# IsseiMori/lajolla_public

Hardware: AMD Instinct MI355X
Metric: Msamples/sec (whole node), cbox 256spp (higher is better)
Workload: dtype f32; 1 GPU; cbox.xml 512x512 @ 256 spp, path integrator (Lambertian + area light, max_depth -1, rr_depth 5); rng=pcg32, one stream per (pixel, sample), seed 0x853c49e6748fea9b, parallelism=1 GPU, collective=none

## Files before the change

### __graft_entry__.py

```python
import os
import sys

ROOT = os.path.dirname(os.path.abspath(__file__))
if ROOT not in sys.path:
    sys.path.insert(0, ROOT)


def build():
    from lajolla_public_amd import build as b
    lib = b.build_product()
    b.build_oracle()
    b.build_twin()
    b.build_twin_tile()
    b.build_reference_subset()
    import lajolla_public_amd as lj
    lj.load_library()
    assert os.path.exists(lib)


def smoke():
    import numpy as np
    sys.path.insert(0, os.path.join(ROOT, "tests"))
    import lajolla_public_amd as lj
    from helpers import Oracle, random_rays, scene_path
    hs = lj.parse_scene(scene_path("cbox"))
    ctx = lj.Context(0)
    sc = lj.Scene(ctx, hs)
    o = Oracle(hs)
    rays = random_rays(hs, 20000, 3, o)
    hg, ho = lj.intersect(sc, rays["org"], rays["dir"], 0.0, np.inf), o.intersect(rays)
    for f in ("t", "u", "v", "shape_id", "prim_id"):
        assert np.array_equal(hg[f].view(np.uint32), ho[f].view(np.uint32)), f"traversal mismatch in {f}"
    crop, spp = (224, 232, 288, 280), 8
    rc, _, ps, _ = o.render(spp=spp, rng_mode=0, crop=crop, per_sample=True)
    pg = lj.render_samples(sc, crop, spp=spp)
    rel = np.abs(pg - ps).max(axis=-1) / np.maximum(np.abs(ps).max(axis=-1), 1e-3)
    assert rc == 0 and np.median(rel) < 2e-6 and (rel > 1e-3).mean() < 0.02, (np.median(rel), (rel > 1e-3).mean())
    assert abs(pg.mean() / ps.mean() - 1) < 5e-4
    st = sc.stats()
    print(f"smoke ok: {st.samples} samples, K={st.bounce_iterations / st.samples:.3f}, median rel diff {np.median(rel):.2e}, "
          f"diverged {100 * (rel > 1e-3).mean():.2f} %")


if __name__ == "__main__":
    build()
    if len(sys.argv) > 1 and sys.argv[1] == "smoke":
# ... 2 lines not shown
```

### lajolla_public_amd/build.py

```python
import os
import subprocess
import sys
from concurrent.futures import ThreadPoolExecutor

ROOT = os.path.dirname(os.path.dirname(os.path.abspath(__file__)))
CSRC = os.path.join(ROOT, "lajolla_public_amd", "csrc")
_VARIANT = os.environ.get("LJ_VARIANT", "")
BUILD = os.path.join(ROOT, "build" + ("_" + _VARIANT if _VARIANT else ""))
LIB = os.path.join(ROOT, "lajolla_public_amd", "liblajolla_hip" + ("_" + _VARIANT if _VARIANT else "") + ".so")
_SAN = bool(os.environ.get("LJ_SANITIZE"))
_SAN_FLAGS = ["-fsanitize=address,undefined", "-fno-omit-frame-pointer", "-g"] if _SAN else []
ORACLE_LIB = os.path.join(ROOT, "oracle", "_build", "liblj_oracle_asan.so" if _SAN else "liblj_oracle.so")
TWIN_LIB = os.path.join(ROOT, "tests", "twin", "_build", "libljtwin_asan.so" if _SAN else "libljtwin.so")

HOST_SOURCES = ["host/api_host.cpp", "host/scene_xml.cpp", "host/mesh_io.cpp", "host/image_io.cpp", "host/jpeg_decode.cpp", "host/exr_decode.cpp", "host/png_decode.cpp", "host/tga_bmp_decode.cpp", "host/flatten.cpp", "host/bvh.cpp"]
HIP_SOURCES = ["device/kernels.hip", "device/extend8.hip", "device/volpath.hip", "device/api_device.hip", "device/queries.hip", "device/mega.hip", "device/group.hip", "device/tile.hip"]
ARCH = "gfx950"


def _hipcc():
    for c in (os.environ.get("HIPCC"), "/opt/rocm/bin/hipcc", "hipcc"):
        if c and (os.path.isabs(c) and os.path.exists(c) or not os.path.isabs(c)):
            return c
    raise RuntimeError("hipcc not found")
# ... 85 lines not shown


def build_twin(verbose=True):
    src = os.path.join(ROOT, "tests", "twin", "twin.cpp")
    if not os.path.exists(src):
        return None
    os.makedirs(os.path.dirname(TWIN_LIB), exist_ok=True)
    deps = [src] + _headers() + [os.path.join(CSRC, s) for s in ("host/flatten.cpp", "host/bvh.cpp")]
    if _stale(TWIN_LIB, deps):
        if verbose:
            print("[build] compiling the host twin of the device headers (CPU-side tests only)", file=sys.stderr)
        _run(["g++", "-std=c++17", "-O1" if _SAN else "-O2", "-ffp-contract=off"] + _SAN_FLAGS + _host_fma_flag() + ["-fPIC", "-shared", "-Wall", "-Wno-unused-function",
              "-o", TWIN_LIB, src, os.path.join(CSRC, "host/flatten.cpp"), os.path.join(CSRC, "host/bvh.cpp"), "-lpthread"])
    return TWIN_LIB


TWIN_TILE_LIB = os.path.join(ROOT, "tests", "twin_tile", "_build", "libljtwintile_asan.so" if _SAN else "libljtwintile.so")


def build_twin_tile(verbose=True):
    src = os.path.join(ROOT, "tests", "twin_tile", "twin_tile.cpp")
    if not os.path.exists(src):
        return None
    os.makedirs(os.path.dirname(TWIN_TILE_LIB), exist_ok=True)
    deps = [src] + _headers() + [os.path.join(CSRC, s) for s in ("host/flatten.cpp", "host/bvh.cpp")]
    if _stale(TWIN_TILE_LIB, deps):
        if verbose:
            print("[build] compiling the host twin of the per-tile schedule (CPU-side tests only)", file=sys.stderr)
        _run(["g++", "-std=c++17", "-O1" if _SAN else "-O2", "-ffp-contract=off"] + _SAN_FLAGS + _host_fma_flag() + ["-fPIC", "-shared", "-Wall", "-Wno-unused-function",
              "-o", TWIN_TILE_LIB, src, os.path.join(CSRC, "host/flatten.cpp"), os.path.join(CSRC, "host/bvh.cpp"), "-lpthread"])
    return TWIN_TILE_LIB


def build_reference_subset():
    script = os.path.join(ROOT, "oracle", "ref_build.sh")
    if os.path.isdir(os.environ.get("LJ_REFERENCE_ROOT", "/root/reference")):
        _run(["bash", script])


if __name__ == "__main__":
    build_product()
    if "--oracle" in sys.argv or "--all" in sys.argv:
        build_oracle()
    if "--twin" in sys.argv or "--all" in sys.argv:
        build_twin()
        build_twin_tile()
    print(LIB)
```

### lajolla_public_amd/csrc/device/api_device.hip

```cpp
#include "api_internal.h"

namespace {

void set_device(lj_context *ctx) { HIP_CHECK(hipSetDevice(ctx->device)); }

ljd::DQueue carve_queue(void *base, uint32_t cap) {
    ljd::DQueue q{};
    ljd::Rec4 *p = (ljd::Rec4 *)base;
    auto take = [&]() { ljd::Rec4 *r = p; p += cap; return r; };
    q.ro = take(); q.rd = take(); q.rs = take(); q.rh = take(); q.rw = take(); q.rl = take(); q.rn = take(); q.rg = take();
    return q;
}
size_t queue_bytes(uint32_t cap) { return (size_t)cap * kQueueSlotBytes; }

void ensure_queues(lj_context *ctx, uint32_t cap) {
    if (ctx->queue_capacity >= cap) return;
    cap = (cap + 63u) & ~63u;
    ctx->queue_mem.alloc(queue_bytes(cap));
    ctx->queue_capacity = cap;
}

int *ensure_spill(lj_context *ctx, int levels, uint32_t grid) {
    if (levels <= 0) return nullptr;
    const size_t need = (size_t)levels * grid * 256 * sizeof(int);
// ... 162 lines not shown
            ljd::launch_volpath(ds, pass, (uint32_t)total, (uint32_t *)ctx->chunk_counter.p, sc->ecfg, sc->scfg.variant,
                                 (sc->feat_kinds & ~7u) == 0u && !sc->feat_textured && !sc->feat_envmap && !sc->feat_sphere_lights,
                                ensure_spill(ctx, sc->ecfg.spill_levels, (uint32_t)grid), grid, stream);
            HIP_CHECK(hipGetLastError());
            st.samples += total; st.wavefront_steps++;
            if (rgb_dev) ljd::launch_resolve(pass, (uint32_t)np, rgb_dev, stream);
            if (samples_host) {
                HIP_CHECK(hipMemcpyAsync(samples_host + p0 * (uint64_t)plan.spp * 3, ctx->sample_rgb.p, total * 12, hipMemcpyDeviceToHost, stream));
                HIP_CHECK(hipStreamSynchronize(stream));
            }
        }
        HIP_CHECK(hipEventRecord(ctx->ev_end, stream));
        HIP_CHECK(hipEventSynchronize(ctx->ev_end));
        float ms = 0; HIP_CHECK(hipEventElapsedTime(&ms, ctx->ev_begin, ctx->ev_end));
        unsigned long long nb = 0;
        HIP_CHECK(hipMemcpy(&nb, ctx->chunk_counter.p, 8, hipMemcpyDeviceToHost));
        st.render_ms = ms; st.bounce_iterations = nb;
        if (getenv("LJ_VOLPATH_STATS")) {
            unsigned long long h[32];
            HIP_CHECK(hipMemcpy(h, ctx->chunk_counter.p, sizeof(h), hipMemcpyDeviceToHost));
            const char *names[8] = {"node iterations", "leaf steps", "closest calls", "tracking (bounce ray)", "tracking (shadow segment)", "shadow segments", "path steps", "-"};
            for (int k = 0; k < 7; k++) fprintf(stderr, "[volpath stats] %-26s wave events %12llu  lanes active %5.1f %%  per sample %.2f\n", names[k], h[2 + 2 * k], h[2 + 2 * k] ? 100.0 * h[3 + 2 * k] / (64.0 * h[2 + 2 * k]) : 0.0, (double)h[3 + 2 * k] / (double)st.samples);
        }
        return;
    }
    const size_t mega_lds = ljd::mega_smem(sc->dscene, sc->scfg);
    const bool mega_off = getenv("LJ_TUNE_MEGA") && atoi(getenv("LJ_TUNE_MEGA")) == 0;
    if (mega_lds > 0 && !mega_off) {
        const uint64_t pass_samples_max = pix_per_pass * (uint64_t)plan.spp;
        if (ctx->sample_rgb.bytes < pass_samples_max * 12) ctx->sample_rgb.alloc(pass_samples_max * 12);
        if (!ctx->mega_state.p) ctx->mega_state.alloc(64);
        upload_pixel_list(ctx, plan, stream);
        HIP_CHECK(hipEventRecord(ctx->ev_begin, stream));
        int per_cu = ljd::mega_blocks_per_cu(sc->scfg);
        if (const char *e = getenv("LJ_TUNE_MEGA_BLOCKS_PER_CU")) per_cu = std::max(1, atoi(e));
        uint32_t grab_max = 768, grab_min = 192;
        bool grab_fixed = false;
        if (const char *e = getenv("LJ_TUNE_MEGA_GRAB")) { grab_max = (uint32_t)std::max(64, atoi(e)) & ~63u; grab_fixed = true; }
        double mega_ms = 0;
        unsigned long long hstats[5] = {};
        for (uint64_t p0 = 0; p0 < n_pix; p0 += pix_per_pass) {
            const uint64_t np = std::min<uint64_t>(pix_per_pass, n_pix - p0);
            const uint64_t total = np * (uint64_t)plan.spp;
            ljd::DPass pass{};
            pass.pixel_list = (const uint32_t *)ctx->pixel_list.p + p0; pass.n_pixels = (uint32_t)np; ljd::set_pass_divisors(pass, (uint32_t)plan.spp, (uint32_t)sc->flat.cam.width);
            pass.seed = plan.seed; pass.sample_rgb = (float *)ctx->sample_rgb.p;
            HIP_CHECK(hipMemsetAsync(ctx->mega_state.p, 0, 64, stream));
            uint32_t grab = grab_max;
            if (!grab_fixed) {
                uint64_t draws = 16;
                if (const char *e = getenv("LJ_TUNE_MEGA_DRAWS")) draws = (uint64_t)std::max(1, atoi(e));
                const uint64_t waves = (uint64_t)ctx->n_cus * per_cu * 4, per_draw = total / (waves * draws);
                grab = (uint32_t)std::min<uint64_t>(grab_max, std::max<uint64_t>(grab_min, per_draw & ~(uint64_t)63));
            }
            const uint64_t pieces = (total + grab - 1) / grab;
            const int grid = (int)std::max<uint64_t>(1, std::min<uint64_t>((uint64_t)ctx->n_cus * per_cu, (pieces + 3) / 4));
            if (timing) HIP_CHECK(hipEventRecord(ctx->ev_k0, stream));
            ljd::launch_mega(ds, pass, sc->scfg, sc->flat.n_spheres > 0, (uint32_t)total, grab, (uint32_t *)ctx->mega_state.p,
                             (unsigned long long *)((char *)ctx->mega_state.p + 8), grid, stream);
            HIP_CHECK(hipGetLastError());
            if (timing) {
                HIP_CHECK(hipEventRecord(ctx->ev_k1, stream)); HIP_CHECK(hipEventSynchronize(ctx->ev_k1));
                float a = 0; HIP_CHECK(hipEventElapsedTime(&a, ctx->ev_k0, ctx->ev_k1)); mega_ms += a;
            }
            st.mega_launches++; st.wavefront_steps++;
            if (rgb_dev) ljd::launch_resolve(pass, (uint32_t)np, rgb_dev, stream);
            unsigned long long *h = ctx->stats_host;
// ... 394 lines not shown
```

### lajolla_public_amd/csrc/device/api_internal.h

```cpp
#pragma once
#include <hip/hip_runtime.h>
#include "../host/api_common.h"
#include "../host/flatten.h"
#include "dtypes.h"
#include "dconfig.h"
#include <algorithm>
#include <cstdlib>
#include <cstring>
#include <memory>
#include <string>
#include <vector>

namespace ljd {
ShadeConfig shade_config(size_t n_prims, size_t n_materials, size_t n_lights, size_t n_light_tris, size_t n_light_tri_cdf, size_t n_images3, size_t n_images1, size_t n_env_marg);
int shade_variant(uint32_t kinds, bool textured, bool envmap, bool sphere_lights);
ExtendConfig extend_config(int n_nodes, int n_prims, int bvh_depth, int n_spheres, int n_nodes8, int bvh8_depth, bool open_scene);
int max_stack_depth();
void launch_extend(const DScene &sc, const DQueue &q, const DBlockState *blocks, uint32_t grid, uint32_t seg, uint32_t *work, const uint32_t *chunk_list, uint32_t parity, const ExtendConfig &cfg, int *spill, unsigned long long *stats, hipStream_t s);
bool shade_sorts_segments(const ShadeConfig &cfg);
void launch_shade(const DScene &sc, const DPass &pass, const DQueue &q, const DQueue &qo, uint32_t *sort_perm, uint8_t *sort_keys, DBlockState *blocks, uint32_t n_blocks, uint32_t seg, const ShadeConfig &cfg, uint32_t *work, uint32_t *chunk_list, uint32_t parity, uint32_t extend_waves, hipStream_t s);
void launch_resolve(const DPass &pass, uint32_t n_pixels, float *rgb, hipStream_t s);
size_t tail_smem(const ExtendConfig &ecfg, const ShadeConfig &scfg);
void launch_tail(const DScene &sc, const DPass &pass, const DQueue &q, DBlockState *blocks, uint32_t n_blocks, uint32_t seg, const ExtendConfig &ecfg, const ShadeConfig &scfg, int *spill, hipStream_t s);
void launch_aux(const DScene &sc, const uint32_t *pixel_list, uint32_t n_pixels, int integrator, float *rgb, const ExtendConfig &cfg, int *spill, int grid, hipStream_t s);
void launch_volpath(const DScene &sc, const DPass &pass, uint32_t n_samples, uint32_t *counters, const ExtendConfig &cfg, int shade_variant, bool plain, int *spill, int grid, hipStream_t s);
int volpath_blocks_per_cu(const DScene &sc);
void launch_trace_rays(const DScene &sc, const void *rays, long long n, void *hits, unsigned char *occ, const ExtendConfig &cfg, int *spill, int grid, hipStream_t s);
size_t mega_smem(const DScene &sc, const ShadeConfig &scfg);
int mega_blocks_per_cu(const ShadeConfig &scfg);
void launch_mega(const DScene &sc, const DPass &pass, const ShadeConfig &scfg, bool spheres, uint32_t n_samples, uint32_t grab, uint32_t *sample_counter, unsigned long long *stats, int grid, hipStream_t s);
void launch_trace_rays_scan(const DScene &sc, const void *rays, long long n, void *hits, unsigned char *occ, int grid, hipStream_t s);
size_t tile_cursor_bytes(bool vol);
void launch_tile_init(bool vol, void *cursors, const uint32_t *tiles, uint32_t n_tiles, uint64_t seed, hipStream_t s);
int tile_grid(uint32_t n_tiles, uint32_t lanes);
void launch_tile(bool vol, const DScene &sc, const DTileJob &job, void *cursors, uint32_t lanes, uint32_t budget, uint32_t *alive, const ExtendConfig &cfg, int *spill, hipStream_t s);
void tile_cursor_stats(bool vol, const void *cursors_host, uint32_t n, unsigned long long out[5]);
}

using lj::LjError;

#define HIP_CHECK(expr) do { hipError_t _e = (expr); if (_e != hipSuccess) \
    throw LjError(LJ_ERR_DEVICE, std::string(#expr) + " failed: " + hipGetErrorString(_e)); } while (0)

struct DevBuf {
    void *p = nullptr; size_t bytes = 0;
    void alloc(size_t n) { release(); if (n) { HIP_CHECK(hipMalloc(&p, n)); bytes = n; } }
    void release() { if (p) { (void)hipFree(p); p = nullptr; bytes = 0; } }
    ~DevBuf() { release(); }
    DevBuf() = default; DevBuf(const DevBuf &) = delete; DevBuf &operator=(const DevBuf &) = delete;
};

template <typename T> inline void upload(DevBuf &b, const std::vector<T> &v, hipStream_t s) {
    b.alloc(((std::max<size_t>(v.size(), 1) * sizeof(T)) + 31) & ~(size_t)15);
    if (!v.empty()) HIP_CHECK(hipMemcpyAsync(b.p, v.data(), v.size() * sizeof(T), hipMemcpyHostToDevice, s));
}

static constexpr size_t kQueueSlotBytes = 128;
static constexpr uint32_t kMaxBlocks = 8192;

static constexpr uint32_t kMaxLanes = 8;
struct lj_context {
    int device = 0;
// ... 33 lines not shown
```

### lajolla_public_amd/csrc/device/dshade.h

```cpp
#pragma once
#include "dmath.h"
#include "dconfig.h"

namespace ljd {

template <uint32_t KINDS, bool TEXTURED, bool ENVMAP, bool SPHERE_LIGHTS>
struct ShadeFeat {
    static constexpr uint32_t kinds = KINDS;
    static constexpr bool textured = TEXTURED, envmap = ENVMAP, sphere_lights = SPHERE_LIGHTS;
    static constexpr bool kind(int k) { return ((KINDS >> k) & 1u) != 0u; }
};
using FeatAll = ShadeFeat<0x1ffu, true, true, true>;
using FeatLambert = ShadeFeat<0x001u, false, false, false>;
using FeatPlastic = ShadeFeat<0x003u, false, false, true>;
using FeatLambertTex = ShadeFeat<0x001u, true, false, true>;
using FeatClassic = ShadeFeat<0x007u, true, true, true>;
using FeatDisney = ShadeFeat<0x101u, true, true, false>;
template <class Fn> inline void with_shade_variant(int v, Fn &&fn) {
    switch (v) {
        case 0: fn(FeatLambert{}); break;
        case 1: fn(FeatPlastic{}); break;
        case 2: fn(FeatLambertTex{}); break;
        case 3: fn(FeatClassic{}); break;
        case 4: fn(FeatDisney{}); break;
// ... 710 lines not shown
    }
    if (Ft::kind(1) && m.kind == 1) {
        f3 Ks = tex3<Ft>(sc, m, 1, vx), Kd = tex3<Ft>(sc, m, 0, vx);
        float lS = luminance(Ks), lR = luminance(Kd);
        if (lS + lR <= 0.0f) return s;
        float spec_prob = lS / (lS + lR);
        if (rw < spec_prob) {
            float roughness = clampf(tex1<Ft>(sc, m, 2, vx), 0.01f, 1.0f);
            f3 hm = to_world(frame, sample_visible_normals(to_local(frame, dir_in), roughness * roughness, r0, r1));
            s.dir_out = normalize(-dir_in + hm * (2.0f * dot(dir_in, hm)));
            s.roughness = roughness;
        } else s.dir_out = to_world(frame, sample_cos_hemisphere(r0, r1));
        s.valid = true;
        return s;
    }
    return s;
}

LJ_HD bool material_supported(int kind) { return kind >= 0 && kind <= 8; }

struct PathState {
    f3 org, dir;
    float ht, hu, hv; int32_t hcode;
    f3 sdir; float stfar;
    f3 W; float rr, p2;
    f3 rad, nee;
    uint32_t sample; uint64_t rng;
    float eta_scale, spread;
    uint32_t flags;
};

struct ShadeCounters { uint32_t bounces, closest, shadow, done; };

LJ_HD void generate_path(const DScene &sc, const DPass &pass, uint32_t sample_id, PathState &ps) {
    const uint32_t p = fast_div(sample_id, pass.by_spp), s = sample_id - p * pass.spp;
    const uint32_t pixel = pass.pixel_list[p];
    const int y = (int)fast_div(pixel, pass.by_width), x = (int)(pixel - (uint32_t)y * (uint32_t)sc.cam.width);
    const uint64_t stream = (uint64_t)pixel * pass.spp + s;
    const uint64_t inc = pcg32_inc(stream);
    uint64_t st = pcg32_init(stream, pass.seed);
    const float jy = pcg32_real(st, inc);
    const float jx = pcg32_real(st, inc);
    ps.org = ld3(sc.cam.org);
    ps.dir = camera_primary_dir(sc.cam, x, y, jx, jy);
    ps.sdir = mk3(0, 0, 0); ps.stfar = 0.0f;
    ps.W = mk3(1, 1, 1); ps.rr = 1.0f; ps.p2 = -1.0f;
    ps.rad = mk3(0, 0, 0); ps.nee = mk3(0, 0, 0);
    ps.sample = sample_id; ps.rng = st;
    ps.eta_scale = 1.0f; ps.spread = sc.init_spread;
    ps.flags = 2u;
}

template <class Ft, bool DEFER_RR>
LJ_HD bool shade_path_body(const DScene &sc, uint64_t inc, PathState &ps, ShadeCounters &cnt) {
    if (ps.hcode & HIT_VIS_BIT) ps.rad = ps.rad + ps.nee;
    const bool primary = ps.p2 < 0.0f;
    if (ps.flags & PF_NO_EXT) return false;
    const int gprim = (ps.hcode & 0x3fffffff) - 1;
    const uint32_t nv_prev = ps.flags & 0xffffu;
    if (gprim < 0) {
        if (Ft::envmap && sc.envmap_light_id >= 0) {
            const DLight &E = sc.lights[sc.envmap_light_id];
            f3 L = light_emission<Ft>(sc, E, -ps.dir, mk3(0, 0, 0));
            if (primary) ps.rad = ps.rad + L;
            else {
                float p1 = E.pmf * pdf_point_on_light<Ft>(sc, E, mk3(0, 0, 0), -ps.dir, ps.org);
                float p2 = ps.p2;
                float w2 = (p2 * p2) / (p1 * p1 + p2 * p2);
                ps.rad = ps.rad + ps.W * L * w2;
            }
        }
        return false;
    }
    DVertex vx = build_vertex(sc, ps.org, ps.dir, ps.ht, ps.hu, ps.hv, gprim, primary ? ps.spread : 0.0f);
    if (vx.light_id >= 0) {
        const DLight &EL = sc.lights[vx.light_id];
        f3 L = light_emission<Ft>(sc, EL, -ps.dir, vx.gn);
        if (primary) ps.rad = ps.rad + L;
        else {
            f3 dv = vx.position - ps.org;
            float G = fabsf(dot(ps.dir, vx.gn)) / dot(dv, dv);
            float p2 = ps.p2 * G;
            float p1 = EL.pmf * pdf_point_on_light<Ft>(sc, EL, vx.position, vx.gn, ps.org);
// ... 80 lines not shown
```

### lajolla_public_amd/csrc/device/mega.hip

```cpp
#include "dstage.h"
#include "dtrace.h"
#include "dconfig.h"

namespace ljd {

#define LJ_CONST __attribute__((address_space(4)))

constexpr uint32_t kItemCap = 512;
constexpr uint32_t kWaveScanBytes = 64 * 48 + 64 * 8 + 64 * 4 + kItemCap * 2;

struct ScanCtx {
    const LJ_CONST float *boxes;
    int n_used;
    const LJ_LDS int *leaf_tab;
    const LJ_LDS v4f *lprims; int prim_stride;
    const DSphere *spheres;
    LJ_LDS v4f *rays;
    LJ_LDS unsigned long long *keys;
    LJ_LDS uint32_t *occl;
    LJ_LDS uint16_t *items;
};

__device__ __forceinline__ uint32_t lane_id() { return __builtin_amdgcn_mbcnt_hi(~0u, __builtin_amdgcn_mbcnt_lo(~0u, 0u)); }

struct ScanRay { float ix, iy, iz, ox, oy, oz; };
__device__ __forceinline__ ScanRay scan_ray(f3 org, f3 dir) {
    const float tiny = 1e-18f;
    const float dx = fabsf(dir.x) < tiny ? copysignf(tiny, dir.x) : dir.x, dy = fabsf(dir.y) < tiny ? copysignf(tiny, dir.y) : dir.y,
                dz = fabsf(dir.z) < tiny ? copysignf(tiny, dir.z) : dir.z;
    ScanRay r;
    r.ix = __builtin_amdgcn_rcpf(dx); r.iy = __builtin_amdgcn_rcpf(dy); r.iz = __builtin_amdgcn_rcpf(dz);
    r.ox = org.x * r.ix; r.oy = org.y * r.iy; r.oz = org.z * r.iz;
    return r;
}
template <bool FAR>
__device__ __forceinline__ float scan_box(const float (&b)[6], const ScanRay &r, float tnear, float tfar) {
    const float ax = __builtin_fmaf(b[0], r.ix, -r.ox), bx = __builtin_fmaf(b[3], r.ix, -r.ox);
    const float ay = __builtin_fmaf(b[1], r.iy, -r.oy), by = __builtin_fmaf(b[4], r.iy, -r.oy);
    const float az = __builtin_fmaf(b[2], r.iz, -r.oz), bz = __builtin_fmaf(b[5], r.iz, -r.oz);
    const float te = fmaxf(fmaxf(fminf(ax, bx), fminf(ay, by)), fmaxf(fminf(az, bz), tnear));
    float tx = fminf(fminf(fmaxf(ax, bx), fmaxf(ay, by)), fmaxf(az, bz));
    if (FAR) tx = fminf(tx, tfar);
    return __builtin_fmaf(tx, -1.0000005f, te);
}
__device__ __forceinline__ uint32_t shift_in_sign(uint32_t mask, float d) { return __builtin_amdgcn_alignbit(mask, f2u(d), 31u); }

template <bool E, bool S>
__device__ __forceinline__ void scan_leaf_boxes(const ScanCtx &sx, const ScanRay &re, float tnear_e, const ScanRay &rs, float tnear_s, float tfar_s, uint32_t &me, uint32_t &ms) {
    const int n = sx.n_used;
    int k = 0;
    for (; k + 4 <= n; k += 4) {
        float b[4][6];
#pragma unroll
// ... 7 lines not shown
        }
    }
    for (; k < n; k++) {
        float b[6];
#pragma unroll
        for (int j = 0; j < 6; j++) b[j] = sx.boxes[k * 8 + j];
        if (E) me = shift_in_sign(me, scan_box<false>(b, re, tnear_e, INFINITY));
        if (S) ms = shift_in_sign(ms, scan_box<true>(b, rs, tnear_s, tfar_s));
    }
}
__device__ __forceinline__ void scan_leaf_boxes2(const ScanCtx &sx, f3 org, f3 dir_e, float tnear_e, f3 dir_s, float tnear_s, float tfar_s, bool any_e, bool any_s,
                                                 uint32_t &me, uint32_t &ms) {
    const ScanRay re = scan_ray(org, dir_e), rs = scan_ray(org, dir_s);
    tnear_e = fmaxf(tnear_e, 0.0f); tnear_s = fmaxf(tnear_s, 0.0f);
    me = 0u; ms = 0u;
    if (any_e && any_s) scan_leaf_boxes<true, true>(sx, re, tnear_e, rs, tnear_s, tfar_s, me, ms);
    else if (any_e) scan_leaf_boxes<true, false>(sx, re, tnear_e, rs, tnear_s, tfar_s, me, ms);
    else if (any_s) scan_leaf_boxes<false, true>(sx, re, tnear_e, rs, tnear_s, tfar_s, me, ms);
}

template <bool SPHERES>
__device__ __forceinline__ void scan_trace(const ScanCtx &sx, bool has_e, bool has_s, f3 org, f3 dir_e, float tnear_e, f3 dir_s, float tnear_s, float tfar_s,
                                           float &ht, float &hu, float &hv, int &gprim_out, bool &occluded) {
#pragma clang fp contract(off)
    const uint32_t lane = lane_id();
    uint32_t me = 0, ms = 0;
    scan_leaf_boxes2(sx, org, dir_e, tnear_e, dir_s, tnear_s, tfar_s, __ballot(has_e) != 0ull, __ballot(has_s) != 0ull, me, ms);
    me = has_e ? me : 0u; ms = has_s ? ms : 0u;
    v4f r0, r1, r2;
    r0.x = org.x; r0.y = org.y; r0.z = org.z; r0.w = tfar_s;
    r1.x = dir_e.x; r1.y = dir_e.y; r1.z = dir_e.z; r1.w = tnear_e;
    r2.x = dir_s.x; r2.y = dir_s.y; r2.z = dir_s.z; r2.w = tnear_s;
    sx.rays[lane * 3] = r0; sx.rays[lane * 3 + 1] = r1; sx.rays[lane * 3 + 2] = r2;
    sx.keys[lane] = ~0ull; sx.occl[lane] = 0u;
    for (;;) {
        uint32_t n_items = 0;
        for (;;) {
            const bool has = (ms | me) != 0u;
            const unsigned long long b = __ballot(has);
            if (b == 0ull || n_items + 64u > kItemCap) break;
            if (has) {
                uint32_t leaf, kind;
                if (ms) { leaf = (uint32_t)(sx.n_used - 1) - (uint32_t)__builtin_ctz(ms); ms &= ms - 1u; kind = 1u; }
                else { leaf = (uint32_t)(sx.n_used - 1) - (uint32_t)__builtin_ctz(me); me &= me - 1u; kind = 0u; }
                const uint32_t idx = n_items + __builtin_amdgcn_mbcnt_hi((uint32_t)(b >> 32), __builtin_amdgcn_mbcnt_lo((uint32_t)b, 0u));
                sx.items[idx] = (uint16_t)(lane | (leaf << 6) | (kind << 11));
            }
            n_items += (uint32_t)__popcll(b);
        }
        if (n_items == 0u) break;
        __builtin_amdgcn_fence(__ATOMIC_RELEASE, "wavefront"); __builtin_amdgcn_wave_barrier();
        for (uint32_t r = 0; r < n_items; r += 64u) {
            if (r + lane < n_items) {
                const uint32_t it = sx.items[r + lane];
                const uint32_t src = it & 63u, leaf = (it >> 6) & 31u, kind = it >> 11;
                const v4f o4 = sx.rays[src * 3], d4 = sx.rays[src * 3 + 1 + kind];
                RayF ray;
                ray.ox = o4.x; ray.oy = o4.y; ray.oz = o4.z; ray.dx = d4.x; ray.dy = d4.y; ray.dz = d4.z;
                ray.tnear = d4.w; ray.tfar = kind ? o4.w : INFINITY;
                const int first = sx.leaf_tab[2 * leaf], cnt = sx.leaf_tab[2 * leaf + 1];
                for (int p = 0; p < cnt; p++) {
                    const int pi = first + p, S = sx.prim_stride;
                    const v4f p0 = sx.lprims[pi], p1 = sx.lprims[S + pi], p2 = sx.lprims[2 * S + pi];
                    const int gprim = __float_as_int(p0.w);
                    bool hit; float t;
                    if (!SPHERES || __float_as_int(p1.w) == 0) {
                        const float v0[3] = {p0.x, p0.y, p0.z}, v1[3] = {p1.x, p1.y, p1.z}, v2[3] = {p2.x, p2.y, p2.z};
                        float U, V, Ssum;
                        hit = tri_test_raw(ray, ray.tfar, v0, v1, v2, t, U, V, Ssum);
                    } else {
                        double td = 0.0;
                        hit = sphere_test(ray, sx.spheres[__float_as_int(p2.w)], td);
                        t = (float)td;
                    }
                    if (hit) {
                        if (kind) sx.occl[src] = 1u;
                        else (void)__hip_atomic_fetch_min(&sx.keys[src], ((unsigned long long)f2u(t) << 32) | (unsigned long long)(((uint32_t)gprim << 16) | (uint32_t)pi), __ATOMIC_RELAXED, __HIP_MEMORY_SCOPE_WAVEFRONT);
                    }
                }
            }
        }
        __builtin_amdgcn_fence(__ATOMIC_RELEASE, "wavefront"); __builtin_amdgcn_wave_barrier();
        if (__ballot((ms | me) != 0u) == 0ull) break;
    }
    const unsigned long long key = sx.keys[lane];
    const uint32_t low = (uint32_t)key;
    occluded = sx.occl[lane] != 0u;
    gprim_out = -1; ht = 0.0f; hu = 0.0f; hv = 0.0f;
    if (has_e && low != 0xffffffffu) {
        const int pi = (int)(low & 0xffffu), S = sx.prim_stride;
        gprim_out = (int)(low >> 16);
        ht = u2f((uint32_t)(key >> 32));
        const v4f p0 = sx.lprims[pi], p1 = sx.lprims[S + pi], p2 = sx.lprims[2 * S + pi];
        if (!SPHERES || __float_as_int(p1.w) == 0) {
            RayF ray;
            ray.ox = org.x; ray.oy = org.y; ray.oz = org.z; ray.dx = dir_e.x; ray.dy = dir_e.y; ray.dz = dir_e.z; ray.tnear = tnear_e; ray.tfar = INFINITY;
            const float v0[3] = {p0.x, p0.y, p0.z}, v1[3] = {p1.x, p1.y, p1.z}, v2[3] = {p2.x, p2.y, p2.z};
            float t, U, V, Ssum;
            (void)tri_test_raw(ray, INFINITY, v0, v1, v2, t, U, V, Ssum);
            const float rS = div_ieee(1.0f, Ssum);
            hu = U * rS; hv = V * rS;
        }
    }
}

__device__ __forceinline__ f3 add_rounded(f3 a, f3 b) {
#pragma clang fp contract(off)
    return mk3(a.x + b.x, a.y + b.y, a.z + b.z);
}

__device__ __forceinline__ void opaque(float &x) { asm volatile("" : "+v"(x)); }
__device__ __forceinline__ void opaque(f3 &v) { opaque(v.x); opaque(v.y); opaque(v.z); }
__device__ __forceinline__ void opaque_state(PathState &ps) {
    opaque(ps.org); opaque(ps.dir); opaque(ps.ht); opaque(ps.hu); opaque(ps.hv); opaque(ps.sdir); opaque(ps.stfar);
    opaque(ps.W); opaque(ps.rr); opaque(ps.p2); opaque(ps.rad); opaque(ps.nee); opaque(ps.eta_scale); opaque(ps.spread);
}

__device__ __forceinline__ ScanCtx stage_scan(const DScene &sc, uint32_t at) {
    ScanCtx sx;
    char *base = (char *)lj_smem + at;
    LJ_LDS int *lt = (LJ_LDS int *)base;
    for (int i = threadIdx.x; i < sc.n_scan_leaves; i += kBlock) { lt[2 * i] = sc.scan_leaves[i].first; lt[2 * i + 1] = sc.scan_leaves[i].count; }
    const uint32_t lt_bytes = ((uint32_t)sc.n_scan_leaves * 8u + 15u) & ~15u;
    LJ_LDS v4f *lp = (LJ_LDS v4f *)(base + lt_bytes);
    const v4f *src = reinterpret_cast<const v4f *>(sc.leaf_prims);
    for (int i = threadIdx.x; i < sc.n_prims * 3; i += kBlock) lp[(i % 3) * sc.n_prims + (i / 3)] = src[i];
    char *wave = base + lt_bytes + (uint32_t)sc.n_prims * 48u + (threadIdx.x >> 6) * kWaveScanBytes;
    sx.boxes = (const LJ_CONST float *)(uintptr_t)sc.scan_leaves; sx.n_used = sc.n_scan_used;
    sx.leaf_tab = lt; sx.lprims = lp; sx.prim_stride = sc.n_prims; sx.spheres = sc.spheres;
    sx.rays = (LJ_LDS v4f *)wave; sx.keys = (LJ_LDS unsigned long long *)(wave + 64 * 48); sx.occl = (LJ_LDS uint32_t *)(wave + 64 * 48 + 64 * 8);
    sx.items = (LJ_LDS uint16_t *)(wave + 64 * 48 + 64 * 8 + 64 * 4);
    return sx;
}
size_t scan_smem(int n_scan_leaves, int n_prims) { return (((size_t)n_scan_leaves * 8 + 15) & ~(size_t)15) + (size_t)n_prims * 48 + 4 * (size_t)kWaveScanBytes; }

#ifndef LJ_MEGA_OCC
#define LJ_MEGA_OCC 5
#endif
template <class Ft> struct MegaOccupancy { static constexpr int waves = 3; };
template <> struct MegaOccupancy<FeatLambert> { static constexpr int waves = LJ_MEGA_OCC; };
#ifndef LJ_MEGA_OCC_PLASTIC
#define LJ_MEGA_OCC_PLASTIC 4
#endif
template <> struct MegaOccupancy<FeatPlastic> { static constexpr int waves = LJ_MEGA_OCC_PLASTIC; };

template <class Ft, bool SPHERES>
__global__ void __launch_bounds__(kBlock, MegaOccupancy<Ft>::waves) k_mega(DScene sc, DPass pass, ShadeStage stg, uint32_t scan_at, uint32_t n_samples, uint32_t grab,
                                                              uint32_t *sample_counter, unsigned long long *stats) {
    stage_shade_tables<2>(sc, stg, 0u);
    const ScanCtx sx = stage_scan(sc, scan_at);
    __syncthreads();
    const uint32_t lane = lane_id();
    ShadeCounters cnt; cnt.bounces = cnt.closest = cnt.shadow = cnt.done = 0;
    uint32_t steps = 0;
    bool live = false, exhausted = false;
    uint32_t w_next = 0, w_end = 0;
    PathState ps;
    ps.flags = 0u; ps.stfar = 0.0f; ps.sample = 0u;
    for (;;) {
        opaque_state(ps);
        if (live) {
            steps++;
            if (!shade_path<Ft>(sc, pass, ps, cnt)) {
                float *o = pass.sample_rgb + 3ull * ps.sample;
                o[0] = ps.rad.x; o[1] = ps.rad.y; o[2] = ps.rad.z;
                cnt.done++; live = false;
            }
        }
        const unsigned long long dead = __ballot(!live);
        if (dead != 0ull && !exhausted) {
            if (w_next == w_end) {
                uint32_t b = 0;
                if (lane == 0u) b = atomicAdd(sample_counter, grab);
                b = (uint32_t)__builtin_amdgcn_readfirstlane((int)b);
                if (b >= n_samples) exhausted = true;
                else { w_next = b; w_end = (n_samples - b < grab) ? n_samples : b + grab; }
            }
            if (!exhausted) {
                const uint32_t left = w_end - w_next, n_dead = (uint32_t)__popcll(dead);
                const uint32_t rank = __builtin_amdgcn_mbcnt_hi((uint32_t)(dead >> 32), __builtin_amdgcn_mbcnt_lo((uint32_t)dead, 0u));
                if (!live && rank < left) { generate_path(sc, pass, w_next + rank, ps); live = true; }
                w_next += n_dead < left ? n_dead : left;
            }
        }
        if (__ballot(live) == 0ull) { if (exhausted) break; else continue; }
        opaque_state(ps);
        const bool has_e = live && !(ps.flags & PF_NO_EXT), has_s = live && ps.stfar > 0.0f;
        float ht, hu, hv; int gprim; bool occluded;
        scan_trace<SPHERES>(sx, has_e, has_s, ps.org, ps.dir, (ps.flags & 0xffffu) == 2u ? 0.0f : sc.eps, ps.sdir, sc.eps, ps.stfar, ht, hu, hv, gprim, occluded);
        if (live) {
            if (has_s && !occluded) ps.rad = add_rounded(ps.rad, ps.nee);
            ps.ht = ht; ps.hu = hu; ps.hv = hv; ps.hcode = gprim + 1;
            if (ps.flags & PF_NO_EXT) {
                float *o = pass.sample_rgb + 3ull * ps.sample;
                o[0] = ps.rad.x; o[1] = ps.rad.y; o[2] = ps.rad.z;
                cnt.done++; live = false;
            }
        }
    }
    const uint32_t b = wave_sum(cnt.bounces), cl = wave_sum(cnt.closest), sh = wave_sum(cnt.shadow), dn = wave_sum(cnt.done), sp = wave_sum(steps);
    if (lane == 0u) {
        atomicAdd(&stats[0], (unsigned long long)b); atomicAdd(&stats[1], (unsigned long long)cl); atomicAdd(&stats[2], (unsigned long long)sh);
        atomicAdd(&stats[3], (unsigned long long)dn); atomicAdd(&stats[4], (unsigned long long)sp);
    }
}

struct RayIO { float org[3]; float tnear; float dir[3]; float tfar; };
struct HitIO { float t, u, v; int32_t shape_id, prim_id; };
__global__ void __launch_bounds__(kBlock) k_trace_rays_scan(DScene sc, const RayIO *rays, long long n, HitIO *hits, unsigned char *occ) {
    const ScanCtx sx = stage_scan(sc, 0u);
    __syncthreads();
    const long long stride = (long long)gridDim.x * kBlock;
    for (long long i0 = (long long)blockIdx.x * kBlock; i0 < n; i0 += stride) {
        const long long i = i0 + threadIdx.x;
        const bool act = i < n;
        f3 org = mk3(0, 0, 0), dir = mk3(0, 0, 1); float tn = 0.0f, tf = 0.0f;
        if (act) { org = ld3(rays[i].org); dir = ld3(rays[i].dir); tn = rays[i].tnear; tf = rays[i].tfar; }
        float ht, hu, hv; int gprim; bool occluded;
        if (occ) {
            scan_trace<true>(sx, false, act, org, dir, 0.0f, dir, tn, tf, ht, hu, hv, gprim, occluded);
            if (act) occ[i] = occluded ? 1 : 0;
        } else {
            scan_trace<true>(sx, act, false, org, dir, tn, dir, 0.0f, 0.0f, ht, hu, hv, gprim, occluded);
            if (act) {
                HitIO o; o.t = 0; o.u = 0; o.v = 0; o.shape_id = -1; o.prim_id = -1;
                if (gprim >= 0 && ht <= tf) { const DPrimShade &ps = sc.prims[gprim]; o.t = ht; o.u = hu; o.v = hv; o.shape_id = ps.shape_id; o.prim_id = ps.prim_id; }
                hits[i] = o;
            }
        }
    }
}


size_t mega_smem(const DScene &sc, const ShadeConfig &scfg) {
    if (sc.n_scan_leaves <= 0 || !scfg.stage_prims || scfg.smem == 0) return 0;
    const size_t at = (scfg.smem + 15) & ~(size_t)15, total = at + scan_smem(sc.n_scan_leaves, sc.n_prims);
    return total <= 64 * 1024 ? total : 0;
}

int mega_blocks_per_cu(const ShadeConfig &scfg) {
    int waves = 3;
    with_shade_variant(scfg.variant, [&](auto ft) { waves = MegaOccupancy<decltype(ft)>::waves; });
    return waves;
}

void launch_mega(const DScene &sc, const DPass &pass, const ShadeConfig &scfg, bool spheres, uint32_t n_samples, uint32_t grab, uint32_t *sample_counter,
                 unsigned long long *stats, int grid, hipStream_t s) {
    const ShadeStage st = make_shade_stage(scfg);
    const uint32_t at = (uint32_t)((scfg.smem + 15) & ~(size_t)15);
    const size_t smem = mega_smem(sc, scfg);
    with_shade_variant(scfg.variant, [&](auto ft) {
        using Ft = decltype(ft);
        if (spheres) hipLaunchKernelGGL((k_mega<Ft, true>), dim3(grid), dim3(kBlock), smem, s, sc, pass, st, at, n_samples, grab, sample_counter, stats);
        else hipLaunchKernelGGL((k_mega<Ft, false>), dim3(grid), dim3(kBlock), smem, s, sc, pass, st, at, n_samples, grab, sample_counter, stats);
    });
}

void launch_trace_rays_scan(const DScene &sc, const void *rays, long long n, void *hits, unsigned char *occ, int grid, hipStream_t s) {
    hipLaunchKernelGGL(k_trace_rays_scan, dim3(grid), dim3(kBlock), scan_smem(sc.n_scan_leaves, sc.n_prims), s, sc, (const RayIO *)rays, n, (HitIO *)hits, occ);
}

}
```

Measured before the change: 5496 Msamples/s.

## Stash precomputed camera samples in LDS for mega kernel path regeneration

```diff
diff --git a/__graft_entry__.py b/__graft_entry__.py
--- a/__graft_entry__.py
+++ b/__graft_entry__.py
@@ -12,6 +12,7 @@
     b.build_oracle()
     b.build_twin()
     b.build_twin_tile()
+    b.build_twin_regen()
     b.build_reference_subset()
     import lajolla_public_amd as lj
     lj.load_library()
diff --git a/lajolla_public_amd/build.py b/lajolla_public_amd/build.py
--- a/lajolla_public_amd/build.py
+++ b/lajolla_public_amd/build.py
@@ -141,6 +141,21 @@
     return TWIN_TILE_LIB
 
 
+TWIN_REGEN_LIB = os.path.join(ROOT, "tests", "twin_regen", "_build", "libljtwinregen_asan.so" if _SAN else "libljtwinregen.so")
+
+
+def build_twin_regen(verbose=True):
+    src = os.path.join(ROOT, "tests", "twin_regen", "twin_regen.cpp")
+    if not os.path.exists(src):
+        return None
+    os.makedirs(os.path.dirname(TWIN_REGEN_LIB), exist_ok=True)
+    if _stale(TWIN_REGEN_LIB, [src] + _headers()):
+        if verbose:
+            print("[build] compiling the host model of the mega kernel's sample bookkeeping (CPU-side tests only)", file=sys.stderr)
+        _run(["g++", "-std=c++17", "-O1" if _SAN else "-O2"] + _SAN_FLAGS + ["-fPIC", "-shared", "-Wall", "-Wno-unused-function", "-o", TWIN_REGEN_LIB, src])
+    return TWIN_REGEN_LIB
+
+
 def build_reference_subset():
     script = os.path.join(ROOT, "oracle", "ref_build.sh")
     if os.path.isdir(os.environ.get("LJ_REFERENCE_ROOT", "/root/reference")):
@@ -154,4 +169,5 @@
     if "--twin" in sys.argv or "--all" in sys.argv:
         build_twin()
         build_twin_tile()
+        build_twin_regen()
     print(LIB)
diff --git a/lajolla_public_amd/csrc/device/api_device.hip b/lajolla_public_amd/csrc/device/api_device.hip
--- a/lajolla_public_amd/csrc/device/api_device.hip
+++ b/lajolla_public_amd/csrc/device/api_device.hip
@@ -218,7 +218,7 @@
         if (!ctx->mega_state.p) ctx->mega_state.alloc(64);
         upload_pixel_list(ctx, plan, stream);
         HIP_CHECK(hipEventRecord(ctx->ev_begin, stream));
-        int per_cu = ljd::mega_blocks_per_cu(sc->scfg);
+        int per_cu = ljd::mega_blocks_per_cu(sc->dscene, sc->scfg);
         if (const char *e = getenv("LJ_TUNE_MEGA_BLOCKS_PER_CU")) per_cu = std::max(1, atoi(e));
         uint32_t grab_max = 768, grab_min = 192;
         bool grab_fixed = false;
diff --git a/lajolla_public_amd/csrc/device/api_internal.h b/lajolla_public_amd/csrc/device/api_internal.h
--- a/lajolla_public_amd/csrc/device/api_internal.h
+++ b/lajolla_public_amd/csrc/device/api_internal.h
@@ -27,7 +27,7 @@
 int volpath_blocks_per_cu(const DScene &sc);
 void launch_trace_rays(const DScene &sc, const void *rays, long long n, void *hits, unsigned char *occ, const ExtendConfig &cfg, int *spill, int grid, hipStream_t s);
 size_t mega_smem(const DScene &sc, const ShadeConfig &scfg);
-int mega_blocks_per_cu(const ShadeConfig &scfg);
+int mega_blocks_per_cu(const DScene &sc, const ShadeConfig &scfg);
 void launch_mega(const DScene &sc, const DPass &pass, const ShadeConfig &scfg, bool spheres, uint32_t n_samples, uint32_t grab, uint32_t *sample_counter, unsigned long long *stats, int grid, hipStream_t s);
 void launch_trace_rays_scan(const DScene &sc, const void *rays, long long n, void *hits, unsigned char *occ, int grid, hipStream_t s);
 size_t tile_cursor_bytes(bool vol);
diff --git a/lajolla_public_amd/csrc/device/dregen.h b/lajolla_public_amd/csrc/device/dregen.h
--- /dev/null
+++ b/lajolla_public_amd/csrc/device/dregen.h
@@ -0,0 +1,36 @@
+#pragma once
+#include "dtypes.h"
+
+namespace ljd {
+
+constexpr uint32_t kRegenSlots = 64;
+
+struct RegenState { uint32_t w_next, w_end, st_base, st_fill, st_read; bool exhausted; };
+
+LJ_HD void regen_init(RegenState &rg) { rg.w_next = rg.w_end = rg.st_base = rg.st_fill = rg.st_read = 0u; rg.exhausted = false; }
+
+LJ_HD uint32_t regen_take(RegenState &rg, uint32_t n_dead, uint32_t &first) {
+    const uint32_t have = rg.st_fill - rg.st_read, take = n_dead < have ? n_dead : have;
+    first = rg.st_read;
+    rg.st_read += take;
+    return take;
+}
+
+LJ_HD bool regen_needs_grab(const RegenState &rg) { return rg.w_next == rg.w_end && !rg.exhausted; }
+
+LJ_HD void regen_grabbed(RegenState &rg, uint32_t b, uint32_t n_samples, uint32_t grab) {
+    if (b >= n_samples) rg.exhausted = true;
+    else { rg.w_next = b; rg.w_end = (n_samples - b < grab) ? n_samples : b + grab; }
+}
+
+LJ_HD uint32_t regen_refill(RegenState &rg) {
+    const uint32_t left = rg.w_end - rg.w_next, n_gen = left < kRegenSlots ? left : kRegenSlots;
+    if (n_gen == 0u || rg.st_read != rg.st_fill) return 0u;
+    rg.st_base = rg.w_next; rg.st_fill = n_gen; rg.st_read = 0u;
+    rg.w_next += n_gen;
+    return n_gen;
+}
+
+LJ_HD bool regen_done(const RegenState &rg) { return rg.exhausted && rg.w_next == rg.w_end && rg.st_read == rg.st_fill; }
+
+}
diff --git a/lajolla_public_amd/csrc/device/dshade.h b/lajolla_public_amd/csrc/device/dshade.h
--- a/lajolla_public_amd/csrc/device/dshade.h
+++ b/lajolla_public_amd/csrc/device/dshade.h
@@ -766,7 +766,7 @@
 
 struct ShadeCounters { uint32_t bounces, closest, shadow, done; };
 
-LJ_HD void generate_path(const DScene &sc, const DPass &pass, uint32_t sample_id, PathState &ps) {
+LJ_HD void camera_sample(const DScene &sc, const DPass &pass, uint32_t sample_id, f3 &dir, uint64_t &rng) {
     const uint32_t p = fast_div(sample_id, pass.by_spp), s = sample_id - p * pass.spp;
     const uint32_t pixel = pass.pixel_list[p];
     const int y = (int)fast_div(pixel, pass.by_width), x = (int)(pixel - (uint32_t)y * (uint32_t)sc.cam.width);
@@ -775,14 +775,23 @@
     uint64_t st = pcg32_init(stream, pass.seed);
     const float jy = pcg32_real(st, inc);
     const float jx = pcg32_real(st, inc);
+    dir = camera_primary_dir(sc.cam, x, y, jx, jy);
+    rng = st;
+}
+LJ_HD void start_path(const DScene &sc, uint32_t sample_id, f3 dir, uint64_t rng, PathState &ps) {
     ps.org = ld3(sc.cam.org);
-    ps.dir = camera_primary_dir(sc.cam, x, y, jx, jy);
+    ps.dir = dir;
     ps.sdir = mk3(0, 0, 0); ps.stfar = 0.0f;
     ps.W = mk3(1, 1, 1); ps.rr = 1.0f; ps.p2 = -1.0f;
     ps.rad = mk3(0, 0, 0); ps.nee = mk3(0, 0, 0);
-    ps.sample = sample_id; ps.rng = st;
+    ps.sample = sample_id; ps.rng = rng;
     ps.eta_scale = 1.0f; ps.spread = sc.init_spread;
     ps.flags = 2u;
+}
+LJ_HD void generate_path(const DScene &sc, const DPass &pass, uint32_t sample_id, PathState &ps) {
+    f3 dir; uint64_t rng;
+    camera_sample(sc, pass, sample_id, dir, rng);
+    start_path(sc, sample_id, dir, rng, ps);
 }
 
 template <class Ft, bool DEFER_RR>
diff --git a/lajolla_public_amd/csrc/device/mega.hip b/lajolla_public_amd/csrc/device/mega.hip
--- a/lajolla_public_amd/csrc/device/mega.hip
+++ b/lajolla_public_amd/csrc/device/mega.hip
@@ -1,13 +1,17 @@
 #include "dstage.h"
 #include "dtrace.h"
 #include "dconfig.h"
+#include "dregen.h"
 
 namespace ljd {
 
 #define LJ_CONST __attribute__((address_space(4)))
 
-constexpr uint32_t kItemCap = 512;
-constexpr uint32_t kWaveScanBytes = 64 * 48 + 64 * 8 + 64 * 4 + kItemCap * 2;
+constexpr uint32_t kItemCap = 512, kItemCapTight = 304;
+constexpr uint32_t kWaveStashBytes = kRegenSlots * (8 + 12);
+constexpr uint32_t wave_scan_bytes(uint32_t item_cap, bool stash) { return 64 * 48 + 64 * 8 + (stash ? kWaveStashBytes : 0u) + 64 + item_cap * 2; }
+static_assert(wave_scan_bytes(kItemCap, false) % 16 == 0 && wave_scan_bytes(kItemCapTight, true) % 16 == 0, "the next wave's rays are 16-byte records");
+constexpr size_t kLdsPerCU = 160 * 1024, kLdsGranule = 320 * 4;
 
 struct ScanCtx {
     const LJ_CONST float *boxes;
@@ -17,8 +21,10 @@
     const DSphere *spheres;
     LJ_LDS v4f *rays;
     LJ_LDS unsigned long long *keys;
-    LJ_LDS uint32_t *occl;
-    LJ_LDS uint16_t *items;
+    LJ_LDS uint8_t *occl;
+    LJ_LDS uint16_t *items; uint32_t item_cap;
+    LJ_LDS uint64_t *st_rng;
+    LJ_LDS float *st_dir;
 };
 
 __device__ __forceinline__ uint32_t lane_id() { return __builtin_amdgcn_mbcnt_hi(~0u, __builtin_amdgcn_mbcnt_lo(~0u, 0u)); }
@@ -92,13 +98,13 @@
     r1.x = dir_e.x; r1.y = dir_e.y; r1.z = dir_e.z; r1.w = tnear_e;
     r2.x = dir_s.x; r2.y = dir_s.y; r2.z = dir_s.z; r2.w = tnear_s;
     sx.rays[lane * 3] = r0; sx.rays[lane * 3 + 1] = r1; sx.rays[lane * 3 + 2] = r2;
-    sx.keys[lane] = ~0ull; sx.occl[lane] = 0u;
+    sx.keys[lane] = ~0ull; sx.occl[lane] = 0;
     for (;;) {
         uint32_t n_items = 0;
         for (;;) {
             const bool has = (ms | me) != 0u;
             const unsigned long long b = __ballot(has);
-            if (b == 0ull || n_items + 64u > kItemCap) break;
+            if (b == 0ull || n_items + 64u > sx.item_cap) break;
             if (has) {
                 uint32_t leaf, kind;
                 if (ms) { leaf = (uint32_t)(sx.n_used - 1) - (uint32_t)__builtin_ctz(ms); ms &= ms - 1u; kind = 1u; }
@@ -134,7 +140,7 @@
                         t = (float)td;
                     }
                     if (hit) {
-                        if (kind) sx.occl[src] = 1u;
+                        if (kind) sx.occl[src] = 1;
                         else (void)__hip_atomic_fetch_min(&sx.keys[src], ((unsigned long long)f2u(t) << 32) | (unsigned long long)(((uint32_t)gprim << 16) | (uint32_t)pi), __ATOMIC_RELAXED, __HIP_MEMORY_SCOPE_WAVEFRONT);
                     }
                 }
@@ -176,6 +182,12 @@
     opaque(ps.W); opaque(ps.rr); opaque(ps.p2); opaque(ps.rad); opaque(ps.nee); opaque(ps.eta_scale); opaque(ps.spread);
 }
 
+__device__ __forceinline__ void stash_start(const DScene &sc, const ScanCtx &sx, uint32_t st_base, uint32_t slot, PathState &ps) {
+    const f3 dir = mk3(sx.st_dir[slot], sx.st_dir[64 + slot], sx.st_dir[128 + slot]);
+    start_path(sc, st_base + slot, dir, sx.st_rng[slot], ps);
+}
+
+template <uint32_t ITEM_CAP, bool STASH>
 __device__ __forceinline__ ScanCtx stage_scan(const DScene &sc, uint32_t at) {
     ScanCtx sx;
     char *base = (char *)lj_smem + at;
@@ -185,14 +197,16 @@
     LJ_LDS v4f *lp = (LJ_LDS v4f *)(base + lt_bytes);
     const v4f *src = reinterpret_cast<const v4f *>(sc.leaf_prims);
     for (int i = threadIdx.x; i < sc.n_prims * 3; i += kBlock) lp[(i % 3) * sc.n_prims + (i / 3)] = src[i];
-    char *wave = base + lt_bytes + (uint32_t)sc.n_prims * 48u + (threadIdx.x >> 6) * kWaveScanBytes;
+    char *wave = base + lt_bytes + (uint32_t)sc.n_prims * 48u + (threadIdx.x >> 6) * wave_scan_bytes(ITEM_CAP, STASH);
     sx.boxes = (const LJ_CONST float *)(uintptr_t)sc.scan_leaves; sx.n_used = sc.n_scan_used;
     sx.leaf_tab = lt; sx.lprims = lp; sx.prim_stride = sc.n_prims; sx.spheres = sc.spheres;
-    sx.rays = (LJ_LDS v4f *)wave; sx.keys = (LJ_LDS unsigned long long *)(wave + 64 * 48); sx.occl = (LJ_LDS uint32_t *)(wave + 64 * 48 + 64 * 8);
-    sx.items = (LJ_LDS uint16_t *)(wave + 64 * 48 + 64 * 8 + 64 * 4);
+    sx.rays = (LJ_LDS v4f *)wave; sx.keys = (LJ_LDS unsigned long long *)(wave + 64 * 48);
+    sx.st_rng = (LJ_LDS uint64_t *)(wave + 64 * 48 + 64 * 8); sx.st_dir = (LJ_LDS float *)(wave + 64 * 48 + 64 * 8 + kRegenSlots * 8);
+    const uint32_t after = 64 * 48 + 64 * 8 + (STASH ? kWaveStashBytes : 0u);
+    sx.occl = (LJ_LDS uint8_t *)(wave + after); sx.items = (LJ_LDS uint16_t *)(wave + after + 64); sx.item_cap = ITEM_CAP;
     return sx;
 }
-size_t scan_smem(int n_scan_leaves, int n_prims) { return (((size_t)n_scan_leaves * 8 + 15) & ~(size_t)15) + (size_t)n_prims * 48 + 4 * (size_t)kWaveScanBytes; }
+size_t scan_smem(int n_scan_leaves, int n_prims, uint32_t item_cap = kItemCap, bool stash = false) { return (((size_t)n_scan_leaves * 8 + 15) & ~(size_t)15) + (size_t)n_prims * 48 + 4 * (size_t)wave_scan_bytes(item_cap, stash); }
 
 #ifndef LJ_MEGA_OCC
 #define LJ_MEGA_OCC 5
@@ -203,18 +217,27 @@
 #define LJ_MEGA_OCC_PLASTIC 4
 #endif
 template <> struct MegaOccupancy<FeatPlastic> { static constexpr int waves = LJ_MEGA_OCC_PLASTIC; };
+#ifndef LJ_MEGA_STASH
+#define LJ_MEGA_STASH 1
+#endif
+template <class Ft> constexpr bool mega_stash() { return LJ_MEGA_STASH && MegaOccupancy<Ft>::waves >= 5; }
+#ifndef LJ_MEGA_ITEM_CAP_TIGHT
+#define LJ_MEGA_ITEM_CAP_TIGHT 0
+#endif
+template <class Ft> constexpr uint32_t mega_item_cap() { return (mega_stash<Ft>() || (LJ_MEGA_ITEM_CAP_TIGHT && MegaOccupancy<Ft>::waves >= 5)) ? kItemCapTight : kItemCap; }
 
 template <class Ft, bool SPHERES>
 __global__ void __launch_bounds__(kBlock, MegaOccupancy<Ft>::waves) k_mega(DScene sc, DPass pass, ShadeStage stg, uint32_t scan_at, uint32_t n_samples, uint32_t grab,
                                                               uint32_t *sample_counter, unsigned long long *stats) {
     stage_shade_tables<2>(sc, stg, 0u);
-    const ScanCtx sx = stage_scan(sc, scan_at);
+    constexpr bool STASH = mega_stash<Ft>();
+    const ScanCtx sx = stage_scan<mega_item_cap<Ft>(), STASH>(sc, scan_at);
     __syncthreads();
     const uint32_t lane = lane_id();
     ShadeCounters cnt; cnt.bounces = cnt.closest = cnt.shadow = cnt.done = 0;
     uint32_t steps = 0;
-    bool live = false, exhausted = false;
-    uint32_t w_next = 0, w_end = 0;
+    bool live = false;
+    RegenState rg; regen_init(rg);
     PathState ps;
     ps.flags = 0u; ps.stfar = 0.0f; ps.sample = 0u;
     for (;;) {
@@ -228,22 +251,51 @@
             }
         }
         const unsigned long long dead = __ballot(!live);
-        if (dead != 0ull && !exhausted) {
-            if (w_next == w_end) {
-                uint32_t b = 0;
-                if (lane == 0u) b = atomicAdd(sample_counter, grab);
-                b = (uint32_t)__builtin_amdgcn_readfirstlane((int)b);
-                if (b >= n_samples) exhausted = true;
-                else { w_next = b; w_end = (n_samples - b < grab) ? n_samples : b + grab; }
-            }
-            if (!exhausted) {
-                const uint32_t left = w_end - w_next, n_dead = (uint32_t)__popcll(dead);
-                const uint32_t rank = __builtin_amdgcn_mbcnt_hi((uint32_t)(dead >> 32), __builtin_amdgcn_mbcnt_lo((uint32_t)dead, 0u));
-                if (!live && rank < left) { generate_path(sc, pass, w_next + rank, ps); live = true; }
-                w_next += n_dead < left ? n_dead : left;
-            }
-        }
-        if (__ballot(live) == 0ull) { if (exhausted) break; else continue; }
+        if constexpr (STASH) {
+            uint32_t n_dead = (uint32_t)__popcll(dead);
+            if (n_dead != 0u) {
+                uint32_t rank = __builtin_amdgcn_mbcnt_hi((uint32_t)(dead >> 32), __builtin_amdgcn_mbcnt_lo((uint32_t)dead, 0u));
+                uint32_t first;
+                uint32_t take = regen_take(rg, n_dead, first);
+                if (!live && rank < take) { stash_start(sc, sx, rg.st_base, first + rank, ps); live = true; }
+                n_dead -= take; rank -= take;
+                if (n_dead != 0u) {
+                    if (regen_needs_grab(rg)) {
+                        uint32_t b = 0;
+                        if (lane == 0u) b = atomicAdd(sample_counter, grab);
+                        regen_grabbed(rg, (uint32_t)__builtin_amdgcn_readfirstlane((int)b), n_samples, grab);
+                    }
+                    const uint32_t n_gen = regen_refill(rg);
+                    if (n_gen != 0u) {
+                        __builtin_amdgcn_fence(__ATOMIC_RELEASE, "wavefront"); __builtin_amdgcn_wave_barrier();
+                        if (lane < n_gen) {
+                            f3 dir; uint64_t rng;
+                            camera_sample(sc, pass, rg.st_base + lane, dir, rng);
+                            sx.st_rng[lane] = rng; sx.st_dir[lane] = dir.x; sx.st_dir[64 + lane] = dir.y; sx.st_dir[128 + lane] = dir.z;
+                        }
+                        __builtin_amdgcn_fence(__ATOMIC_RELEASE, "wavefront"); __builtin_amdgcn_wave_barrier();
+                        take = regen_take(rg, n_dead, first);
+                        if (!live && rank < take) { stash_start(sc, sx, rg.st_base, first + rank, ps); live = true; }
+                    }
+                }
+            }
+            if (__ballot(live) == 0ull) break;
+        } else {
+            if (dead != 0ull && !rg.exhausted) {
+                if (rg.w_next == rg.w_end) {
+                    uint32_t b = 0;
+                    if (lane == 0u) b = atomicAdd(sample_counter, grab);
+                    regen_grabbed(rg, (uint32_t)__builtin_amdgcn_readfirstlane((int)b), n_samples, grab);
+                }
+                if (!rg.exhausted) {
+                    const uint32_t left = rg.w_end - rg.w_next, n_dead = (uint32_t)__popcll(dead);
+                    const uint32_t rank = __builtin_amdgcn_mbcnt_hi((uint32_t)(dead >> 32), __builtin_amdgcn_mbcnt_lo((uint32_t)dead, 0u));
+                    if (!live && rank < left) { generate_path(sc, pass, rg.w_next + rank, ps); live = true; }
+                    rg.w_next += n_dead < left ? n_dead : left;
+                }
+            }
+            if (__ballot(live) == 0ull) { if (rg.exhausted) break; else continue; }
+        }
         opaque_state(ps);
         const bool has_e = live && !(ps.flags & PF_NO_EXT), has_s = live && ps.stfar > 0.0f;
         float ht, hu, hv; int gprim; bool occluded;
@@ -268,7 +320,7 @@
 struct RayIO { float org[3]; float tnear; float dir[3]; float tfar; };
 struct HitIO { float t, u, v; int32_t shape_id, prim_id; };
 __global__ void __launch_bounds__(kBlock) k_trace_rays_scan(DScene sc, const RayIO *rays, long long n, HitIO *hits, unsigned char *occ) {
-    const ScanCtx sx = stage_scan(sc, 0u);
+    const ScanCtx sx = stage_scan<kItemCap, false>(sc, 0u);
     __syncthreads();
     const long long stride = (long long)gridDim.x * kBlock;
     for (long long i0 = (long long)blockIdx.x * kBlock; i0 < n; i0 += stride) {
@@ -294,14 +346,18 @@
 
 size_t mega_smem(const DScene &sc, const ShadeConfig &scfg) {
     if (sc.n_scan_leaves <= 0 || !scfg.stage_prims || scfg.smem == 0) return 0;
-    const size_t at = (scfg.smem + 15) & ~(size_t)15, total = at + scan_smem(sc.n_scan_leaves, sc.n_prims);
+    uint32_t item_cap = kItemCap; bool stash = false;
+    with_shade_variant(scfg.variant, [&](auto ft) { item_cap = mega_item_cap<decltype(ft)>(); stash = mega_stash<decltype(ft)>(); });
+    const size_t at = (scfg.smem + 15) & ~(size_t)15, total = at + scan_smem(sc.n_scan_leaves, sc.n_prims, item_cap, stash);
     return total <= 64 * 1024 ? total : 0;
 }
 
-int mega_blocks_per_cu(const ShadeConfig &scfg) {
+int mega_blocks_per_cu(const DScene &sc, const ShadeConfig &scfg) {
     int waves = 3;
     with_shade_variant(scfg.variant, [&](auto ft) { waves = MegaOccupancy<decltype(ft)>::waves; });
-    return waves;
+    const size_t smem = (mega_smem(sc, scfg) + kLdsGranule - 1) / kLdsGranule * kLdsGranule;
+    const int by_lds = smem ? (int)(kLdsPerCU / smem) : waves;
+    return waves < by_lds ? waves : by_lds;
 }
 
 void launch_mega(const DScene &sc, const DPass &pass, const ShadeConfig &scfg, bool spheres, uint32_t n_samples, uint32_t grab, uint32_t *sample_counter,
```

Measured after the change: 5785 Msamples/s (median of 6 runs). 5.3% higher.
